# watsonyanghx/GAN_Lib_Tensorflow

Measured on AMD Instinct MI355X. Metric: images/sec (G+D step) SNGAN-ResNet CIFAR-10 bs=64, higher is better.
Workload: dtype bf16; 1 GPU; SNGAN ResNet CIFAR-10 32x32 bs=64 hinge: 1 G update (2x64 fakes) + 5 D updates (64 real + 64 fake) per step; global_batch=64, per_gpu_batch=64, parallelism=dp1, graphs=True, finite=True, collectives_in_graphs=False, grad_wire=fp32

## Files before the change

### gan_lib_tensorflow_amd/csrc/conv_igemm.hip

```cpp
#include "gank_common.h"
#ifdef GANK_TUNING
static __device__ int gank_stats_dbg = 0;
static void gank_stats_dbg_init() {
  static const int v = gank_tune("GANK_STATS_DBG", 0);
  static bool done = false;
  if (!done) { done = true; if (v) (void)hipMemcpyToSymbol(HIP_SYMBOL(gank_stats_dbg), &v, sizeof(int)); }
}
#else
static inline void gank_stats_dbg_init() {}
#endif
#include <stdlib.h>
#include <type_traits>

#ifndef GANK_KMODE
#define GANK_KMODE 0
#endif
#define IG_IN_ZEROINS2X 16
#define IG_IN_STRIDE2 32
#define IG_RES_UP2X 128

struct IgemmArgs {
  const bf16* x;
  const bf16* w;
  const float* bias;
  const bf16* res;
  const bf16* mask;
  bf16* y;
  int N, H, W;
  int Hin, Win;
  int Cin, Cout, CoutPad, Kpad;
  int ks, pad, taps;
  int M;
  int flags;
  float scale;
  int nsteps;
  int tiles_m, tiles_n;
  int shw, sw;
  int korder;
  int tiles_pp;
  float* stat_sums;
  int stat_n_per_group, stat_groups, stat_prezeroed;
  int phase_inner;
  const float* cbn_stats;
  const float* cbn_gamma;
  const float* cbn_beta;
  const int* cbn_labels;
  int cbn_n_per_group, cbn_n_labels;
  bf16* aux_out;
};

static int phase_inner_env() {
  static const int v = gank_tune("GANK_PHASE_INNER", 1);
  return v;
}

constexpr int LROW = 72;

template <int CTRL>
__device__ __forceinline__ float pp_dpp_add(float v) {
  return v + __builtin_bit_cast(float, __builtin_amdgcn_update_dpp(0, __builtin_bit_cast(int, v), CTRL, 0xF, 0xF, false));
}
__device__ __forceinline__ float pp_row_sum(float v) {
  v = pp_dpp_add<0xB1>(v);
  v = pp_dpp_add<0x4E>(v);
  v = pp_dpp_add<0x141>(v);
  v = pp_dpp_add<0x140>(v);
  return v;
}

template <bool WANT_D>
__device__ __forceinline__ void epi_tile_wide(const f32x16& acc, float scale, const float* __restrict__ bias, const bf16* __restrict__ mask_px,
                                              const bf16* __restrict__ res_px, bf16* __restrict__ y_px, int h, bool otanh, float (*d)[8]) {
#pragma unroll
  for (int q = 0; q < 2; q++) {
    const int c = 16 * q + 8 * h;
    float v[8];
    acc_widen(acc, q, scale, v);
    float bb[8] = {0.f, 0.f, 0.f, 0.f, 0.f, 0.f, 0.f, 0.f};
    if (bias) {
      const f32x4 b0 = *reinterpret_cast<const f32x4*>(bias + c), b1 = *reinterpret_cast<const f32x4*>(bias + c + 4);
#pragma unroll
      for (int e = 0; e < 4; e++) { bb[e] = b0[e]; bb[4 + e] = b1[e]; }
    }
#pragma unroll
    for (int e = 0; e < 8; e++) {
      if constexpr (WANT_D) d[q][e] = v[e];
      v[e] += bb[e];
    }
    if (mask_px) {
      const bf16x8 mk = *reinterpret_cast<const bf16x8*>(mask_px + c);
#pragma unroll
      for (int e = 0; e < 8; e++) {
        const bool on = bf2f(mk[e]) > 0.f;
        v[e] = on ? v[e] : 0.f;
        if constexpr (WANT_D) d[q][e] = on ? d[q][e] : -bb[e];
      }
    }
    if (res_px) {
      const bf16x8 rs = *reinterpret_cast<const bf16x8*>(res_px + c);
#pragma unroll
      for (int e = 0; e < 8; e++) {
        const float t = bf2f(rs[e]);
        v[e] += t;
        if constexpr (WANT_D) d[q][e] += t;
      }
    }
    bf16x8 out;
#pragma unroll
    for (int e = 0; e < 8; e++) out[e] = f2bf(otanh ? tanhf(v[e]) : v[e]);
    *reinterpret_cast<bf16x8*>(y_px + c) = out;
  }
}

template <int WM, int WN, int TM, int TN, bool PACKED, int PF, int MODE, bool STATS = false>
__global__ __launch_bounds__(WM* WN * 64) void conv_igemm_kernel(IgemmArgs a) {
  static_assert(!STATS || (!PACKED && TN * 16 <= 32), "statistics epilogue: plain operands, at most 32 channels per half-wave");
  constexpr int NT = WM * WN * 64;
  constexpr int BM = WM * TM * 32;
  constexpr int BN = WN * TN * 32;
  constexpr int CP = BM * 8 / NT;
  constexpr int CW = BN * 8 / NT;
  static_assert(CP >= 1 && CW >= 1, "tile too small for the thread count");
  static_assert(!PACKED || (PF == 1 && MODE == 0), "the packed path takes its flags at run time");

  extern __shared__ __attribute__((aligned(16))) char smem[];
  bf16* sP = reinterpret_cast<bf16*>(smem);
  bf16* sW = sP + 2 * BM * LROW;

  const int tid = threadIdx.x;
  const int lane = tid & 63, wave = tid >> 6;
  const int wave_m = wave % WM, wave_n = wave / WM;
  const int r = lane & 31, h = lane >> 5;

  const int nwg = a.tiles_m * a.tiles_n;
  const int lid = xcd_remap(blockIdx.x, nwg);
  const int tile_n = lid % a.tiles_n;
  int tile_m = lid / a.tiles_n;
  constexpr bool PHASE = !PACKED && (MODE & 4) != 0;
  int phase = 0;
  if constexpr (PHASE) {
    if (a.phase_inner) { phase = tile_m & 3; tile_m >>= 2; }
    else { phase = tile_m / a.tiles_pp; tile_m -= phase * a.tiles_pp; }
  }
  const int pad_h = PHASE ? 1 - (phase >> 1) : a.pad, pad_w = PHASE ? 1 - (phase & 1) : a.pad;

  const int st = (a.flags & IG_IN_STRIDE2) ? 2 : 1;
  const bool shr = PACKED ? (a.flags & (GANK_IN_UPSAMPLE2X | IG_IN_ZEROINS2X)) != 0 : (MODE & 2) != 0;
  const bool zins = (a.flags & IG_IN_ZEROINS2X) != 0;
  const bool inrelu = PACKED ? (a.flags & GANK_IN_RELU) != 0 : (MODE & 1) != 0;
  const int LH = shr ? 2 * a.Hin : a.Hin, LW = shr ? 2 * a.Win : a.Win;

  int p_base[CP], p_oh[CP], p_ow[CP];
#pragma unroll
  for (int j = 0; j < CP; j++) {
    const int q = tid + NT * j;
    const int m = tile_m * BM + (q >> 3);
    if (m < a.M) {
      int n, oh, ow;
      pix_decomp(m, a.H, a.W, a.shw, a.sw, n, oh, ow);
      p_base[j] = n * a.Hin * a.Win;
      p_oh[j] = oh * st;
      p_ow[j] = ow * st;
    } else {
      p_base[j] = 0;
      p_oh[j] = -(1 << 20);
      p_ow[j] = 0;
    }
  }

  u32x4 rP[PF][CP], rW[PF][CW];

  constexpr int OOB = 0x7FFFFFF0;
  const __amdgpu_buffer_rsrc_t rs_x = __builtin_amdgcn_make_buffer_rsrc(
      const_cast<bf16*>(a.x), 0, a.N * a.Hin * a.Win * a.Cin * 2, 0x00020000);
  const __amdgpu_buffer_rsrc_t rs_w = __builtin_amdgcn_make_buffer_rsrc(
      const_cast<bf16*>(a.w), 0, a.CoutPad * a.Kpad * 2 * (PHASE ? 4 : 1), 0x00020000);
  int p_off[CP];
  int w_off[CW];
#pragma unroll
  for (int j = 0; j < CP; j++)
    p_off[j] = ((p_base[j] + p_oh[j] * a.Win + p_ow[j]) * a.Cin + ((tid + NT * j) & 7) * 8) * 2;
#pragma unroll
  for (int j = 0; j < CW; j++) {
    const int q = tid + NT * j;
    w_off[j] = (((PHASE ? phase * a.CoutPad : 0) + tile_n * BN + (q >> 3)) * a.Kpad + (q & 7) * 8) * 2;
  }

  const int last = a.nsteps - 1;
  int cur = 0, cur_c0 = 0, cur_tap = 0, cur_dh = -pad_h, cur_dw = -pad_w;
  constexpr bool TAP_INNER = (GANK_KMODE & 1) != 0;
  constexpr int W_AUX = (GANK_KMODE >> 1) == 1 ? 2 : ((GANK_KMODE >> 1) == 2 ? 16 : 0);

  auto load_next = [&](u32x4 (&rP)[CP], u32x4 (&rW)[CW]) {
    if constexpr (!PACKED) {
      const int delta = ((cur_dh * a.Win + cur_dw) * a.Cin + cur_c0) * 2;
#pragma unroll
      for (int j = 0; j < CP; j++) {
        const int ih = p_oh[j] + cur_dh, iw = p_ow[j] + cur_dw;
        bool ok = (unsigned)ih < (unsigned)LH && (unsigned)iw < (unsigned)LW;
        int off;
        if constexpr ((MODE & 2) != 0) {
          if (zins) ok = ok && (((ih | iw) & 1) == 0);
          off = ((p_base[j] + (ih >> 1) * a.Win + (iw >> 1)) * a.Cin + cur_c0 + ((tid + NT * j) & 7) * 8) * 2;
        } else {
          off = p_off[j] + delta;
        }
        rP[j] = __builtin_amdgcn_raw_buffer_load_b128(rs_x, ok ? off : OOB, 0, 0);
      }
    } else {
      const int ktot = a.taps * a.Cin;
#pragma unroll
      for (int j = 0; j < CP; j++) {
        const int cc = (tid + NT * j) & 7;
        const int kb = cur * 64 + cc * 8;
        int tap = kb / a.Cin, ci = kb - tap * a.Cin;
        int th = tap / a.ks;
        int dh = th - a.pad, dw = tap - th * a.ks - a.pad;
        bf16x8 v;
#pragma unroll
        for (int e = 0; e < 8; e++) {
          float val = 0.f;
          if (kb + e < ktot) {
            int ih = p_oh[j] + dh, iw = p_ow[j] + dw;
            bool ok = (unsigned)ih < (unsigned)LH && (unsigned)iw < (unsigned)LW;
            if (zins) ok = ok && (((ih | iw) & 1) == 0);
            if (shr) { ih >>= 1; iw >>= 1; }
            if (ok) {
              val = bf2f(a.x[((long)(p_base[j] + ih * a.Win + iw)) * a.Cin + ci]);
              if (inrelu) val = fmaxf(val, 0.f);
            }
          }
          v[e] = f2bf(val);
          if (++ci == a.Cin) {
            ci = 0;
            if (++dw > a.ks - 1 - a.pad) { dw = -a.pad; dh++; }
          }
        }
        rP[j] = __builtin_bit_cast(u32x4, v);
      }
    }
    if constexpr (!PACKED) {
      const int wk = (cur_tap * a.Cin + cur_c0) * 2;
#pragma unroll
      for (int j = 0; j < CW; j++) rW[j] = __builtin_amdgcn_raw_buffer_load_b128(rs_w, w_off[j], wk, W_AUX);
      if (cur < last) {
        cur++;
        if constexpr (TAP_INNER) {
          cur_tap++;
          if (++cur_dw > a.ks - 1 - pad_w) { cur_dw = -pad_w; cur_dh++; }
          if (cur_tap >= a.taps) { cur_tap = 0; cur_dh = -pad_h; cur_dw = -pad_w; cur_c0 += 64; }
        } else {
          cur_c0 += 64;
          if (cur_c0 >= a.Cin) {
            cur_c0 = 0; cur_tap++;
            if (++cur_dw > a.ks - 1 - pad_w) { cur_dw = -pad_w; cur_dh++; }
          }
        }
      }
    } else {
#pragma unroll
      for (int j = 0; j < CW; j++) rW[j] = __builtin_amdgcn_raw_buffer_load_b128(rs_w, w_off[j], cur * 128, 0);
      if (cur < last) cur++;
    }
  };

  auto store_step = [&](int buf, u32x4 (&rP)[CP], u32x4 (&rW)[CW]) {
#pragma unroll
    for (int j = 0; j < CP; j++) {
      const int q = tid + NT * j;
      u32x4 v = rP[j];
      if constexpr (!PACKED && (MODE & 1) != 0) v = relu_bf16x8(v);
      *reinterpret_cast<u32x4*>(sP + (buf * BM + (q >> 3)) * LROW + (q & 7) * 8) = v;
    }
#pragma unroll
    for (int j = 0; j < CW; j++) {
      const int q = tid + NT * j;
      *reinterpret_cast<u32x4*>(sW + (buf * BN + (q >> 3)) * LROW + (q & 7) * 8) = rW[j];
    }
  };

  f32x16 acc[TN][TM];
#pragma unroll
  for (int i = 0; i < TN; i++)
#pragma unroll
    for (int j = 0; j < TM; j++)
#pragma unroll
      for (int e = 0; e < 16; e++) acc[i][j][e] = 0.f;

#pragma unroll
  for (int d = 0; d < PF; d++) load_next(rP[d], rW[d]);
  store_step(0, rP[0], rW[0]);
  __syncthreads();

  auto step = [&](int s, auto slot) {
    constexpr int D = decltype(slot)::value;
    const int buf = s & 1;
    if constexpr (PF > 1) {
      load_next(rP[D], rW[D]);
      if (s + 1 < a.nsteps) store_step(buf ^ 1, rP[(D + 1) % PF], rW[(D + 1) % PF]);
    }
    const bf16* pW = sW + (buf * BN + wave_n * TN * 32 + r) * LROW + h * 8;
    const bf16* pP = sP + (buf * BM + wave_m * TM * 32 + r) * LROW + h * 8;
#pragma unroll
    for (int kk = 0; kk < 4; kk++) {
      bf16x8 fa[TN], fb[TM];
#pragma unroll
      for (int i = 0; i < TN; i++) fa[i] = *reinterpret_cast<const bf16x8*>(pW + i * 32 * LROW + kk * 16);
#pragma unroll
      for (int j = 0; j < TM; j++) fb[j] = *reinterpret_cast<const bf16x8*>(pP + j * 32 * LROW + kk * 16);
#pragma unroll
      for (int i = 0; i < TN; i++)
#pragma unroll
        for (int j = 0; j < TM; j++)
          acc[i][j] = GANK_MFMA32(fa[i], fb[j], acc[i][j]);
    }
    if constexpr (PF == 1) {
      if (s + 1 < a.nsteps) {
        load_next(rP[0], rW[0]);
        store_step(buf ^ 1, rP[0], rW[0]);
      }
    }
    __syncthreads();
  };

  int s0 = 0;
  for (; s0 + PF <= a.nsteps; s0 += PF) {
    if constexpr (PF >= 1) step(s0 + 0, std::integral_constant<int, 0>{});
    if constexpr (PF >= 2) step(s0 + 1, std::integral_constant<int, 1 % PF>{});
    if constexpr (PF >= 3) step(s0 + 2, std::integral_constant<int, 2 % PF>{});
    if constexpr (PF >= 4) step(s0 + 3, std::integral_constant<int, 3 % PF>{});
  }
  if constexpr (PF >= 2) { if (s0 + 0 < a.nsteps) step(s0 + 0, std::integral_constant<int, 0>{}); }
  if constexpr (PF >= 3) { if (s0 + 1 < a.nsteps) step(s0 + 1, std::integral_constant<int, 1 % PF>{}); }
  if constexpr (PF >= 4) { if (s0 + 2 < a.nsteps) step(s0 + 2, std::integral_constant<int, 2 % PF>{}); }

  const bool vec = (a.Cout & 3) == 0;
  const bool wide = (a.Cout & 31) == 0;
  const bool otanh = (a.flags & GANK_OUT_TANH) != 0;
  float st1[STATS ? TN * 16 : 1], st2[STATS ? TN * 16 : 1];
  if constexpr (STATS) {
#pragma unroll
    for (int q = 0; q < TN * 16; q++) { st1[q] = 0.f; st2[q] = 0.f; }
  }
#pragma unroll
  for (int j = 0; j < TM; j++) {
    int m = tile_m * BM + (wave_m * TM + j) * 32 + r;
    if (m >= a.M) continue;
    if constexpr (PHASE) {
      int n_, y_, x_;
      pix_decomp(m, a.H, a.W, a.shw, a.sw, n_, y_, x_);
      m = (n_ * 2 * a.H + 2 * y_ + (phase >> 1)) * 2 * a.W + 2 * x_ + (phase & 1);
    }
    long mr = m;
    if (!PHASE && (a.flags & IG_RES_UP2X)) {
      int n_, y_, x_;
      pix_decomp(m, a.H, a.W, a.shw, a.sw, n_, y_, x_);
      mr = ((long)(n_ * (a.H >> 1) + (y_ >> 1))) * (a.W >> 1) + (x_ >> 1);
    }
    if (wide) {
#pragma unroll
      for (int i = 0; i < TN; i++) {
        const int ct = tile_n * BN + (wave_n * TN + i) * 32;
        float d[2][8];
        epi_tile_wide<STATS>(acc[i][j], a.scale, a.bias ? a.bias + ct : nullptr, a.mask ? a.mask + (long)m * a.Cout + ct : nullptr,
                             a.res ? a.res + mr * a.Cout + ct : nullptr, a.y + (long)m * a.Cout + ct, h, otanh, d);
        if constexpr (STATS) {
#pragma unroll
          for (int q = 0; q < 2; q++)
#pragma unroll
            for (int e = 0; e < 8; e++) { st1[i * 16 + q * 8 + e] += d[q][e]; st2[i * 16 + q * 8 + e] += d[q][e] * d[q][e]; }
        }
      }
      continue;
    }
#pragma unroll
    for (int i = 0; i < TN; i++) {
      const int co0 = tile_n * BN + (wave_n * TN + i) * 32 + 4 * h;
#pragma unroll
      for (int g = 0; g < 4; g++) {
        const int co = co0 + 8 * g;
        if (co >= a.Cout) continue;
        float v[4];
#pragma unroll
        for (int e = 0; e < 4; e++) v[e] = acc[i][j][4 * g + e] * a.scale;
        const long o = (long)m * a.Cout + co;
        if (vec) {
          f32x4 b = {0.f, 0.f, 0.f, 0.f};
          if (a.bias) {
            b = *reinterpret_cast<const f32x4*>(a.bias + co);
#pragma unroll
            for (int e = 0; e < 4; e++) v[e] += b[e];
          }
          if (a.mask) {
            const bf16x4 mk = *reinterpret_cast<const bf16x4*>(a.mask + o);
#pragma unroll
            for (int e = 0; e < 4; e++) v[e] = (bf2f(mk[e]) > 0.f) ? v[e] : 0.f;
          }
          if (a.res) {
            const bf16x4 rs = *reinterpret_cast<const bf16x4*>(a.res + mr * a.Cout + co);
#pragma unroll
            for (int e = 0; e < 4; e++) v[e] += bf2f(rs[e]);
          }
          bf16x4 out;
#pragma unroll
          for (int e = 0; e < 4; e++) out[e] = f2bf(otanh ? tanhf(v[e]) : v[e]);
          *reinterpret_cast<bf16x4*>(a.y + o) = out;
        } else {
#pragma unroll
          for (int e = 0; e < 4; e++) {
            if (co + e >= a.Cout) break;
            float t = v[e];
            if (a.bias) t += a.bias[co + e];
            if (a.mask) t = (bf2f(a.mask[o + e]) > 0.f) ? t : 0.f;
            if (a.res) t += bf2f(a.res[mr * a.Cout + co + e]);
            a.y[o + e] = f2bf(otanh ? tanhf(t) : t);
          }
        }
// ... 968 lines not shown
#pragma unroll
      for (int i = 0; i < 2; i++)
#pragma unroll
        for (int q = 0; q < 2; q++) *reinterpret_cast<bf16x8*>(line + i * 32 + 16 * q) = outl[i][q];
    }
    if constexpr (STATS) {
#pragma unroll
    for (int i = 0; i < 2; i++)
#pragma unroll
      for (int q = 0; q < 2; q++)
#pragma unroll
        for (int e = 0; e < 8; e++) {
          float s1 = pp_row_sum(st1[i][q][e]), s2 = pp_row_sum(st2[i][q][e]);
          s1 += __shfl_xor(s1, 16, 64);
          s2 += __shfl_xor(s2, 16, 64);
          const bool mine = r == (2 * i + q) * 8 + e;
          keep1 = mine ? s1 : keep1;
          keep2 = mine ? s2 : keep2;
        }
    }
  }
  if constexpr (STATS) {
    float* dst = a.stat_sums + ((long)(n / a.stat_n_per_group) * GANK_STAT_SLOTS + (blockIdx.x % GANK_STAT_SLOTS)) * 2 * a.Cout;
    const int ci = r >> 4, cq = (r >> 3) & 1, ce = r & 7;
    const int co = tile_n * 256 + (wn * 2 + ci) * 32 + 16 * cq + 8 * h + ce;
#ifdef GANK_TUNING
    if (gank_stats_dbg) return;
#endif
    atomicAdd(dst + co, keep1);
    atomicAdd(dst + a.Cout + co, keep2);
  }
#endif
}

static thread_local int tl_stats_done = 0;
__global__ void ig_zero_kernel(float* __restrict__ p, int n) {
  const int i = blockIdx.x * blockDim.x + threadIdx.x;
  if (i < n) p[i] = 0.f;
}

static void stats_zero(const IgemmArgs& a, hipStream_t s);
static int t128_min() {
  static const int v = gank_tune("GANK_IGEMM_T128_MIN", 192);
  return v;
}
static bool igemm_stats_ok(const IgemmArgs& a, int BM, int BN) {
  static const int env = gank_tune("GANK_IGEMM_STATS", 1);
  return env && a.stat_sums != nullptr && !(a.flags & GANK_OUT_TANH) && a.M % BM == 0 && a.Cout % BN == 0 &&
         ((long)a.stat_n_per_group * a.H * a.W) % BM == 0;
}
template <int MODE, int PW>
static int launch_pp(const IgemmArgs& a0, hipStream_t s) {
  IgemmArgs a = a0;
  const bool stats = a.stat_sums != nullptr;
  if (stats) { tl_stats_done = 1; stats_zero(a, s); }
  constexpr bool PHASE = (MODE & 4) != 0;
  const int tiles = a.N * (a.H / (256 / PW)) * (a.W / PW);
  a.tiles_pp = tiles;
  a.phase_inner = phase_inner_env();
  a.tiles_m = PHASE ? 4 * tiles : tiles;
  a.tiles_n = a.Cout / 256;
  if (PHASE) { a.Kpad = 4 * a.Cin; a.Hin = a.H; a.Win = a.W; }
  auto kern = stats ? conv_igemm_pp_kernel<MODE, PW, true> : conv_igemm_pp_kernel<MODE, PW, false>;
  if (stats) { GANK_MAX_DYNAMIC_LDS((conv_igemm_pp_kernel<MODE, PW, true>), PP_LDS_BYTES, "conv_igemm_pp"); }
  else { GANK_MAX_DYNAMIC_LDS((conv_igemm_pp_kernel<MODE, PW, false>), PP_LDS_BYTES, "conv_igemm_pp"); }
  static const std::string tag = gank_format("conv_igemm_pp_kernel<%d, %d>", MODE, PW);
  gank_prof_tag(0, tag.c_str());
  hipLaunchKernelGGL(kern, dim3(a.tiles_m * a.tiles_n), dim3(512), PP_LDS_BYTES, s, a);
  GANK_LAUNCH_OK("conv_igemm_pp");
  return 0;
}
static int pp_patch_width(int H, int W) { return (W % 32 == 0 && H % 8 == 0) ? 32 : (W % 16 == 0 && H % 16 == 0) ? 16 : 0; }
static int pp_env() {
  static const int v = gank_tune("GANK_IGEMM_PP", 2);
  return v;
}
static bool pp_enough_blocks(const IgemmArgs& a, int phases) {
  const int pw = pp_patch_width(a.H, a.W);
  return pw != 0 && (long)phases * a.N * (a.H / (256 / pw)) * (a.W / pw) * (a.Cout / 256) >= 224;
}
static bool pp_phase_ok(const IgemmArgs& a) {
  return pp_env() >= 2 && a.Cout % 256 == 0 && a.Cin % 32 == 0 && pp_enough_blocks(a, 4);
}
static int launch_pp_phase(const IgemmArgs& a, hipStream_t s) {
  const bool relu = (a.flags & GANK_IN_RELU) != 0;
  if (pp_patch_width(a.H, a.W) == 32) return relu ? launch_pp<5, 32>(a, s) : launch_pp<4, 32>(a, s);
  return relu ? launch_pp<5, 16>(a, s) : launch_pp<4, 16>(a, s);
}

template <int MODE, int BN>
static int launch_patch(const IgemmArgs& a0, hipStream_t s) {
  IgemmArgs a = a0;
  a.tiles_m = a.N * (a.H / 8) * (a.W / 16);
  a.tiles_n = a.CoutPad / BN;
  const size_t lds = ((size_t)10 * HROWP + (size_t)2 * BN * LROW) * sizeof(bf16);
  auto kern = conv_igemm_patch_kernel<MODE, BN>;
  GANK_MAX_DYNAMIC_LDS(kern, (int)lds, "conv_igemm_patch");
  static const std::string tag = gank_format("conv_igemm_patch_kernel<%d, %d>", MODE, BN);
  gank_prof_tag(0, tag.c_str());
  hipLaunchKernelGGL(kern, dim3(a.tiles_m * a.tiles_n), dim3(256), lds, s, a);
  GANK_LAUNCH_OK("conv_igemm_patch");
  return 0;
}

template <int WM, int WN, int TM, int TN, bool PACKED, int PF, int MODE>
static int launch_cfg(const IgemmArgs& a0, hipStream_t s) {
  IgemmArgs a = a0;
  constexpr int BM = WM * TM * 32, BN = WN * TN * 32;
  a.tiles_m = cdiv(a.M, BM);
  a.tiles_n = a.CoutPad / BN;
  const size_t lds = (size_t)2 * (BM + BN) * LROW * sizeof(bf16);
  static const std::string tag = gank_format("conv_igemm_kernel<%d, %d, %d, %d, %s, %d, %d>", WM, WN, TM, TN, PACKED ? "true" : "false", PF, MODE);
  gank_prof_tag(0, tag.c_str());
  if constexpr (!PACKED && MODE == 0 && TN * 16 <= 32) {
    if (igemm_stats_ok(a, BM, BN)) {
      auto kern = conv_igemm_kernel<WM, WN, TM, TN, PACKED, PF, MODE, true>;
      GANK_MAX_DYNAMIC_LDS(kern, (int)lds, "conv_igemm");
      tl_stats_done = 1;
      stats_zero(a, s);
      hipLaunchKernelGGL(kern, dim3(a.tiles_m * a.tiles_n), dim3(WM * WN * 64), lds, s, a);
      GANK_LAUNCH_OK("conv_igemm");
      return 0;
    }
  }
  auto kern = conv_igemm_kernel<WM, WN, TM, TN, PACKED, PF, MODE>;
  GANK_MAX_DYNAMIC_LDS(kern, (int)lds, "conv_igemm");
  hipLaunchKernelGGL(kern, dim3(a.tiles_m * a.tiles_n), dim3(WM * WN * 64), lds, s, a);
  GANK_LAUNCH_OK("conv_igemm");
  return 0;
}

template <int WM, int WN, int TM, int TN, int PF>
static int launch_phase(const IgemmArgs& a0, hipStream_t s) {
  IgemmArgs a = a0;
  constexpr int BM = WM * TM * 32, BN = WN * TN * 32;
  a.tiles_pp = cdiv(a.M, BM);
  a.phase_inner = phase_inner_env();
  a.tiles_m = 4 * a.tiles_pp;
  a.tiles_n = a.CoutPad / BN;
  const size_t lds = (size_t)2 * (BM + BN) * LROW * sizeof(bf16);
  static const std::string tag = gank_format("conv_igemm_kernel<%d, %d, %d, %d, false, %d, 4>", WM, WN, TM, TN, PF);
  gank_prof_tag(0, tag.c_str());
  if constexpr (TN * 16 <= 32) {
    if (igemm_stats_ok(a, BM, BN)) {
      auto kern = conv_igemm_kernel<WM, WN, TM, TN, false, PF, 4, true>;
      GANK_MAX_DYNAMIC_LDS(kern, (int)lds, "conv_igemm");
      tl_stats_done = 1;
      stats_zero(a, s);
      hipLaunchKernelGGL(kern, dim3(a.tiles_m * a.tiles_n), dim3(WM * WN * 64), lds, s, a);
      GANK_LAUNCH_OK("conv_igemm_phase");
      return 0;
    }
  }
  auto kern = conv_igemm_kernel<WM, WN, TM, TN, false, PF, 4>;
  GANK_MAX_DYNAMIC_LDS(kern, (int)lds, "conv_igemm");
  hipLaunchKernelGGL(kern, dim3(a.tiles_m * a.tiles_n), dim3(WM * WN * 64), lds, s, a);
  GANK_LAUNCH_OK("conv_igemm_phase");
  return 0;
}

template <int WM, int WN, int TM, int TN, int PF>
static int launch_mode(const IgemmArgs& a, hipStream_t s) {
  const int mode = ((a.flags & GANK_IN_RELU) ? 1 : 0) | ((a.flags & (GANK_IN_UPSAMPLE2X | IG_IN_ZEROINS2X)) ? 2 : 0);
  switch (mode) {
    case 0: return launch_cfg<WM, WN, TM, TN, false, PF, 0>(a, s);
    case 1: return launch_cfg<WM, WN, TM, TN, false, PF, 1>(a, s);
    case 2: return launch_cfg<WM, WN, TM, TN, false, PF, 2>(a, s);
    default: return launch_cfg<WM, WN, TM, TN, false, PF, 3>(a, s);
  }
}

int gank_igemm_dispatch(IgemmArgs a, hipStream_t s) {
  GANK_REQUIRE(a.x && a.w && a.y, "conv_igemm: null pointer");
  GANK_REQUIRE(a.N > 0 && a.H > 0 && a.W > 0 && a.Cin > 0 && a.Cout > 0, "conv_igemm: bad shape");
  GANK_REQUIRE(a.ks >= 1 && a.ks <= 7, "conv_igemm: unsupported filter size %d", a.ks);
  GANK_REQUIRE((long)a.N * a.Hin * a.Win * a.Cin < (1L << 30) && (long)a.N * a.H * a.W * a.Cout < (1L << 40), "conv_igemm: tensor too large (32-bit byte offsets)");
  a.taps = a.ks * a.ks;
  a.CoutPad = roundup(a.Cout, 32);
  a.Kpad = roundup(a.taps * a.Cin, 64);
  a.nsteps = a.Kpad / 64;
  a.M = a.N * a.H * a.W;
  a.sw = log2_or_neg(a.W);
  a.shw = log2_or_neg(a.H * a.W);
  const bool packed = (a.Cin % 64) != 0;
  const double flops = 2.0 * a.M * (double)a.Cout * a.taps * a.Cin;
  gank_prof_begin(0, flops, s, 2.0 * ((double)a.N * a.Hin * a.Win * a.Cin + (double)a.taps * a.Cin * a.Cout + (double)a.M * a.Cout +
                                      (a.res ? (double)a.M * a.Cout / ((a.flags & IG_RES_UP2X) ? 4.0 : 1.0) : 0.0) + (a.mask ? (double)a.M * a.Cout : 0.0)));
  int rc;
  const long tiles128 = (long)cdiv(a.M, 128) * (a.CoutPad / 128);
  static const int ko_env = gank_tune("GANK_IGEMM_KORDER", 0);
  a.korder = ko_env;
  static const int pf_env = gank_tune("GANK_IGEMM_PF", 0);
  static const int patch_env = gank_tune("GANK_IGEMM_PATCH", 1);
  const bool patch_geom = patch_env && !packed && a.ks == 3 && a.pad == 1 &&
                          !(a.flags & (GANK_IN_UPSAMPLE2X | IG_IN_ZEROINS2X | IG_IN_STRIDE2)) &&
                          a.W % 16 == 0 && a.H % 8 == 0 && a.Hin == a.H && a.Win == a.W;
  const bool patch_ok = patch_geom && (a.Cout % 4) == 0 && a.CoutPad % 128 == 0;
  const bool patch32_ok = patch_geom && a.CoutPad == 32;
  const bool narrow_ok = !(a.flags & IG_RES_UP2X) && a.Cin == 3 && (a.ks == 1 || a.ks == 3) && a.pad == (a.ks - 1) / 2 && a.CoutPad % 128 == 0 && a.Cout % 4 == 0 &&
                         !(a.flags & (GANK_IN_UPSAMPLE2X | IG_IN_ZEROINS2X | IG_IN_STRIDE2)) && a.Hin == a.H && a.Win == a.W;
  const bool pp_ok = pp_env() && patch_geom && a.Cout % 256 == 0 && a.Kpad == a.taps * a.Cin && pp_enough_blocks(a, 1) &&
                     (pp_env() >= 2 || pp_patch_width(a.H, a.W) == 32);
  if (narrow_ok) {
    rc = a.ks == 3 ? launch_narrow_in<3, 3>(a, s) : launch_narrow_in<1, 3>(a, s);
  } else if (pp_ok) {
    const bool relu = (a.flags & GANK_IN_RELU) != 0;
    if (pp_patch_width(a.H, a.W) == 32) rc = relu ? launch_pp<1, 32>(a, s) : launch_pp<0, 32>(a, s);
    else rc = relu ? launch_pp<1, 16>(a, s) : launch_pp<0, 16>(a, s);
  } else if (patch_ok) {
    rc = (a.flags & GANK_IN_RELU) ? launch_patch<1, 128>(a, s) : launch_patch<0, 128>(a, s);
  } else if (patch32_ok && few_ok(a)) {
    rc = (a.flags & GANK_IN_RELU) ? launch_few<1>(a, s) : launch_few<0>(a, s);
  } else if (patch32_ok) {
    rc = (a.flags & GANK_IN_RELU) ? launch_patch<1, 32>(a, s) : launch_patch<0, 32>(a, s);
  } else if (packed) {
    if (a.CoutPad % 64 == 0) rc = launch_cfg<2, 2, 1, 1, true, 1, 0>(a, s);
    else rc = launch_cfg<4, 1, 2, 1, true, 1, 0>(a, s);
#ifdef GANK_TUNING
  } else if (a.CoutPad % 128 == 0 && tiles128 >= t128_min() && pf_env >= 20) {
    if (pf_env == 20) rc = launch_mode<4, 2, 2, 2, 1>(a, s);
    else if (pf_env == 22 && a.CoutPad % 256 == 0) rc = launch_mode<2, 4, 2, 2, 2>(a, s);
    else if (pf_env == 23 && a.CoutPad % 256 == 0) rc = launch_mode<4, 2, 2, 4, 2>(a, s);
    else rc = launch_mode<4, 2, 2, 2, 2>(a, s);
  } else if (a.CoutPad % 128 == 0 && tiles128 >= t128_min() && (pf_env == 1 || pf_env == 3)) {
    rc = pf_env == 1 ? launch_mode<2, 2, 2, 2, 1>(a, s) : launch_mode<2, 2, 2, 2, 3>(a, s);
  } else if (a.CoutPad % 64 == 0 && !(a.CoutPad % 128 == 0 && tiles128 >= t128_min()) && (pf_env == 1 || pf_env == 11 || pf_env == 12 || pf_env == 3)) {
    rc = (pf_env == 1 || pf_env == 11) ? launch_mode<2, 2, 1, 1, 1>(a, s) : launch_mode<2, 2, 1, 1, 2>(a, s);
#endif
  } else if (a.CoutPad % 128 == 0 && tiles128 >= t128_min()) {
    rc = launch_mode<2, 2, 2, 2, 2>(a, s);
  } else if (a.CoutPad % 64 == 0) {
    rc = launch_mode<2, 2, 1, 1, 4>(a, s);
  } else {
    rc = launch_mode<4, 1, 2, 1, 2>(a, s);
  }
  gank_prof_end(0, s);
  return rc;
}

static int stats_setup(IgemmArgs& a, float* stat_sums, int groups, int N, int Cout, hipStream_t s, int flags) {
  tl_stats_done = 0;
  if (!stat_sums) return 0;
  gank_stats_dbg_init();
  a.stat_prezeroed = (flags & GANK_STATS_PREZEROED) != 0;
  GANK_REQUIRE(groups > 0 && N % groups == 0, "conv statistics: batch %d not divisible by %d towers", N, groups);
  a.stat_sums = stat_sums;
  a.stat_n_per_group = N / groups;
  a.stat_groups = groups;
  return 0;
}
static void stats_zero(const IgemmArgs& a, hipStream_t s) {
  if (a.stat_prezeroed) return;
  const int n = a.stat_groups * GANK_STAT_SLOTS * 2 * a.Cout;
  hipLaunchKernelGGL(ig_zero_kernel, dim3((n + 255) / 256), dim3(256), 0, s, a.stat_sums, n);
}

static int conv2d_fprop_impl(const void* x, const void* wf, const float* bias, const void* residual,
                             const void* relu_ref, void* y, int N, int H, int W, int Cin, int Cout, int ksize,
                             int flags, float scale, float* stat_sums, int groups, void* stream) {
  GANK_REQUIRE(ksize % 2 == 1, "conv2d_fprop: even filter sizes are not on this path (ksize=%d)", ksize);
  GANK_REQUIRE(!(flags & GANK_IN_UPSAMPLE2X) || (H % 2 == 0 && W % 2 == 0), "conv2d_fprop: upsample needs even output size");
  IgemmArgs a{};
  a.x = (const bf16*)x; a.w = (const bf16*)wf; a.bias = bias; a.res = (const bf16*)residual;
  a.mask = (const bf16*)relu_ref; a.y = (bf16*)y;
  a.N = N; a.H = H; a.W = W;
  const bool up = flags & GANK_IN_UPSAMPLE2X;
  a.Hin = up ? H / 2 : H; a.Win = up ? W / 2 : W;
  a.Cin = Cin; a.Cout = Cout; a.ks = ksize; a.pad = (ksize - 1) / 2;
  a.flags = (flags & (GANK_IN_UPSAMPLE2X | GANK_IN_RELU | GANK_OUT_TANH)) |
            ((flags & GANK_RES_UPSAMPLE2X) ? IG_RES_UP2X : 0);
  GANK_REQUIRE(!(flags & GANK_RES_UPSAMPLE2X) || (residual && H % 2 == 0 && W % 2 == 0), "conv2d_fprop: RES_UPSAMPLE2X needs a residual and even output size");
  a.scale = scale;
  if (stats_setup(a, stat_sums, groups, N, Cout, (hipStream_t)stream, flags)) return 1;
  return gank_igemm_dispatch(a, (hipStream_t)stream);
}

extern "C" int gank_conv2d_fprop(const void* x, const void* wf, const float* bias, const void* residual,
                                 const void* relu_ref, void* y, int N, int H, int W, int Cin, int Cout, int ksize,
                                 int flags, float scale, void* stream) {
  return conv2d_fprop_impl(x, wf, bias, residual, relu_ref, y, N, H, W, Cin, Cout, ksize, flags, scale, nullptr, 0, stream);
}
extern "C" int gank_conv2d_fprop_stats(const void* x, const void* wf, const float* bias, const void* residual,
                                       const void* relu_ref, void* y, int N, int H, int W, int Cin, int Cout, int ksize,
                                       int flags, float scale, float* stat_sums, int groups, int* produced, void* stream) {
  GANK_REQUIRE(stat_sums && produced, "conv2d_fprop_stats: null statistics pointers");
  const int rc = conv2d_fprop_impl(x, wf, bias, residual, relu_ref, y, N, H, W, Cin, Cout, ksize, flags, scale, stat_sums, groups, stream);
  *produced = tl_stats_done;
  return rc;
}

extern "C" int gank_cbn_relu_conv3x3_fprop(const void* x, const int32_t* labels, const float* gamma, const float* beta, const float* stats,
                                           const void* wf, const float* bias, void* y, int N, int H, int W, int Cin, int Cout,
                                           int groups, int n_labels, int flags, void* stream) {
  GANK_REQUIRE(x && labels && gamma && beta && stats && wf && y, "cbn_relu_conv3x3_fprop: null pointer");
  GANK_REQUIRE(groups > 0 && N % groups == 0 && n_labels > 0, "cbn_relu_conv3x3_fprop: batch %d / %d towers", N, groups);
  GANK_REQUIRE(Cin % 64 == 0 && W % 16 == 0 && H % 8 == 0, "cbn_relu_conv3x3_fprop: needs Cin %% 64 == 0, W %% 16 == 0, H %% 8 == 0");
  IgemmArgs a{};
// ... 41 lines not shown
  IgemmArgs a{}, b{};
  a.x = (const bf16*)x; a.w = (const bf16*)wf1; a.bias = bias1; a.y = (bf16*)y1;
  a.N = N; a.H = H; a.W = W; a.Hin = H; a.Win = W; a.Cin = 3; a.Cout = Cout1; a.ks = 3; a.pad = 1; a.scale = 1.f;
  a.taps = 9; a.CoutPad = Cout1; a.Kpad = roundup(27, 64); a.nsteps = 1;
  a.M = N * H * W; a.sw = log2_or_neg(W); a.shw = log2_or_neg(H * W);
  a.tiles_m = cdiv(a.M, 128); a.tiles_n = a.CoutPad / 128;
  { static const int ko_env = gank_tune("GANK_IGEMM_KORDER", 0); a.korder = ko_env; }
  const int Hp = H / 2, Wp = W / 2;
  b.x = (const bf16*)x; b.w = (const bf16*)wfs; b.bias = biass; b.y = (bf16*)ys; b.aux_out = (bf16*)pooled;
  b.N = N; b.H = Hp; b.W = Wp; b.Hin = H; b.Win = W; b.Cin = 3; b.Cout = Couts; b.ks = 1; b.pad = 0; b.scale = 1.f;
  b.taps = 1; b.CoutPad = Couts; b.Kpad = roundup(3, 64); b.nsteps = 1;
  b.M = N * Hp * Wp; b.sw = log2_or_neg(Wp); b.shw = log2_or_neg(Hp * Wp);
  b.tiles_m = cdiv(b.M, 128); b.tiles_n = b.CoutPad / 128;
  b.korder = 0;
  hipStream_t s = (hipStream_t)stream;
  const int blocks_a = a.tiles_m * a.tiles_n, blocks_b = b.tiles_m * b.tiles_n;
  gank_prof_begin(0, 2.0 * a.M * (double)Cout1 * 27 + 2.0 * b.M * (double)Couts * 3, s,
                  2.0 * ((double)a.M * 3 + 27.0 * Cout1 + (double)a.M * Cout1 + 3.0 * Couts + (double)b.M * Couts));
  gank_prof_tag(0, "conv_narrow_in_pair_kernel");
  hipLaunchKernelGGL(conv_narrow_in_pair_kernel, dim3(blocks_a + blocks_b), dim3(256), 0, s, a, b, blocks_a);
  gank_prof_end(0, s);
  GANK_LAUNCH_OK("image_conv_pair_fprop");
  return 0;
}

extern "C" int gank_conv2d_dgrad(const void* dy, const void* wd, const void* residual, const void* relu_ref, void* dx,
                                 int N, int H, int W, int Cin, int Cout, int ksize, int flags, float scale, void* stream) {
  GANK_REQUIRE(ksize % 2 == 1, "conv2d_dgrad: even filter sizes are not on this path (ksize=%d)", ksize);
  IgemmArgs a{};
  a.x = (const bf16*)dy; a.w = (const bf16*)wd; a.bias = nullptr; a.res = (const bf16*)residual;
  a.mask = (const bf16*)relu_ref; a.y = (bf16*)dx;
  a.N = N; a.H = H; a.W = W;
  const bool up = flags & GANK_IN_UPSAMPLE2X;
  a.Hin = up ? H / 2 : H; a.Win = up ? W / 2 : W;
  a.Cin = Cout; a.Cout = Cin; a.ks = ksize; a.pad = (ksize - 1) / 2;
  a.flags = (flags & (GANK_IN_UPSAMPLE2X | GANK_IN_RELU));
  a.scale = scale;
  return gank_igemm_dispatch(a, (hipStream_t)stream);
}


extern "C" int gank_conv2d_general_fprop(const void* x, const void* wf, const float* bias, void* y, int N, int Hin, int Win,
                                         int Hout, int Wout, int Cin, int Cout, int ksize, int stride, int pad, int flags, void* stream) {
  GANK_REQUIRE(stride == 1 || stride == 2, "conv2d_general_fprop: stride %d (1 or 2)", stride);
  GANK_REQUIRE(pad >= 0 && pad < ksize, "conv2d_general_fprop: pad %d outside [0, ksize)", pad);
  GANK_REQUIRE(!((flags & GANK_IN_UPSAMPLE2X) && stride == 2), "conv2d_general_fprop: upsampled input with stride 2");
  GANK_REQUIRE(Hin > 0 && Win > 0 && Hout > 0 && Wout > 0, "conv2d_general_fprop: bad sizes");
  IgemmArgs a{};
  a.x = (const bf16*)x; a.w = (const bf16*)wf; a.bias = bias; a.y = (bf16*)y;
  a.N = N; a.H = Hout; a.W = Wout; a.Hin = Hin; a.Win = Win;
  a.Cin = Cin; a.Cout = Cout; a.ks = ksize; a.pad = pad;
  a.flags = (flags & (GANK_IN_UPSAMPLE2X | GANK_IN_RELU | GANK_OUT_TANH)) | (stride == 2 ? IG_IN_STRIDE2 : 0);
  a.scale = 1.f;
  return gank_igemm_dispatch(a, (hipStream_t)stream);
}
extern "C" int gank_conv2d_general_dgrad(const void* dy, const void* wd, const void* relu_ref, void* dx, int N, int Hx, int Wx,
                                         int Hdy, int Wdy, int Cin, int Cout, int ksize, int pad, void* stream) {
  GANK_REQUIRE(pad >= 0 && pad < ksize, "conv2d_general_dgrad: pad %d outside [0, ksize)", pad);
  IgemmArgs a{};
  a.x = (const bf16*)dy; a.w = (const bf16*)wd; a.mask = (const bf16*)relu_ref; a.y = (bf16*)dx;
  a.N = N; a.H = Hx; a.W = Wx; a.Hin = Hdy; a.Win = Wdy;
  a.Cin = Cout; a.Cout = Cin; a.ks = ksize; a.pad = ksize - 1 - pad;
  a.scale = 1.f;
  return gank_igemm_dispatch(a, (hipStream_t)stream);
}

static int upconv3x3_fprop_impl(const void* x, const void* wph, const float* bias, const void* residual, void* y,
                                int N, int Hl, int Wl, int Cin, int Cout, int flags, float* stat_sums, int groups, void* stream) {
  GANK_REQUIRE(Cin % 64 == 0, "upconv3x3_fprop: Cin must be a multiple of 64 (got %d)", Cin);
  IgemmArgs a{};
  a.x = (const bf16*)x; a.w = (const bf16*)wph; a.bias = bias; a.res = (const bf16*)residual; a.y = (bf16*)y;
  a.N = N; a.H = Hl; a.W = Wl; a.Hin = Hl; a.Win = Wl;
  a.Cin = Cin; a.Cout = Cout; a.ks = 2; a.pad = 0;
  a.flags = flags & GANK_OUT_TANH;
  a.scale = 1.f;
  hipStream_t s = (hipStream_t)stream;
  a.taps = 4; a.CoutPad = roundup(Cout, 32); a.Kpad = 4 * Cin; a.nsteps = a.Kpad / 64;
  a.M = N * Hl * Wl; a.sw = log2_or_neg(Wl); a.shw = log2_or_neg(Hl * Wl);
  GANK_REQUIRE((long)N * Hl * Wl * Cin < (1L << 30) && (long)a.M * 4 * Cout < (1L << 31), "upconv3x3_fprop: tensor too large");
  if (stats_setup(a, stat_sums, groups, N, Cout, s, flags)) return 1;
  gank_prof_begin(0, 2.0 * a.M * 4.0 * (double)Cout * 4 * Cin, s, 2.0 * ((double)a.M * Cin + 16.0 * Cin * Cout + 4.0 * a.M * Cout + (residual ? 4.0 * a.M * Cout : 0.0)));
  int rc;
  const long tiles128 = 4L * cdiv(a.M, 128) * (a.CoutPad / 128);
  if (pp_phase_ok(a)) rc = launch_pp_phase(a, s);
  else if (patch_phase_ok(a)) rc = launch_patch_phase<4>(a, s);
  else if (a.CoutPad % 128 == 0 && tiles128 >= t128_min()) rc = launch_phase<2, 2, 2, 2, 2>(a, s);
  else if (a.CoutPad % 64 == 0) rc = launch_phase<2, 2, 1, 1, 4>(a, s);
  else rc = launch_phase<4, 1, 2, 1, 2>(a, s);
  gank_prof_end(0, s);
  return rc;
}

extern "C" int gank_upconv3x3_fprop(const void* x, const void* wph, const float* bias, const void* residual, void* y,
                                    int N, int Hl, int Wl, int Cin, int Cout, int flags, void* stream) {
  return upconv3x3_fprop_impl(x, wph, bias, residual, y, N, Hl, Wl, Cin, Cout, flags, nullptr, 0, stream);
}
extern "C" int gank_upconv3x3_fprop_stats(const void* x, const void* wph, const float* bias, const void* residual, void* y,
                                          int N, int Hl, int Wl, int Cin, int Cout, int flags, float* stat_sums, int groups, int* produced,
                                          void* stream) {
  GANK_REQUIRE(stat_sums && produced, "upconv3x3_fprop_stats: null statistics pointers");
  const int rc = upconv3x3_fprop_impl(x, wph, bias, residual, y, N, Hl, Wl, Cin, Cout, flags, stat_sums, groups, stream);
  *produced = tl_stats_done;
  return rc;
}

extern "C" int gank_upconv3x3_dgrad(const void* dy, const void* wd4, const void* relu_ref, void* dx, int N, int Hl, int Wl,
                                    int Cin, int Cout, void* stream) {
  IgemmArgs a{};
  a.x = (const bf16*)dy; a.w = (const bf16*)wd4; a.mask = (const bf16*)relu_ref; a.y = (bf16*)dx;
  a.N = N; a.H = Hl; a.W = Wl; a.Hin = 2 * Hl; a.Win = 2 * Wl;
  a.Cin = Cout; a.Cout = Cin; a.ks = 4; a.pad = 1;
  a.flags = IG_IN_STRIDE2;
  a.scale = 1.f;
  return gank_igemm_dispatch(a, (hipStream_t)stream);
}

extern "C" int gank_convpool3x3_fprop(const void* x, const void* wp4, const float* bias, const void* residual, void* y,
                                      int N, int Hp, int Wp, int Cin, int Cout, int flags, void* stream) {
  IgemmArgs a{};
  a.x = (const bf16*)x; a.w = (const bf16*)wp4; a.bias = bias; a.res = (const bf16*)residual; a.y = (bf16*)y;
  a.N = N; a.H = Hp; a.W = Wp; a.Hin = 2 * Hp; a.Win = 2 * Wp;
  a.Cin = Cin; a.Cout = Cout; a.ks = 4; a.pad = 1;
  a.flags = IG_IN_STRIDE2 | (flags & GANK_IN_RELU);
  a.scale = 1.f;
  return gank_igemm_dispatch(a, (hipStream_t)stream);
}

extern "C" int gank_convpool3x3_dgrad(const void* dy, const void* wphd, const void* relu_ref, void* dx, int N, int Hp, int Wp,
                                      int Cin, int Cout, void* stream) {
  GANK_REQUIRE(Cout % 64 == 0, "convpool3x3_dgrad: Cout must be a multiple of 64 (got %d)", Cout);
  IgemmArgs a{};
  a.x = (const bf16*)dy; a.w = (const bf16*)wphd; a.mask = (const bf16*)relu_ref; a.y = (bf16*)dx;
  a.N = N; a.H = Hp; a.W = Wp; a.Hin = Hp; a.Win = Wp;
  a.Cin = Cout; a.Cout = Cin; a.ks = 2; a.pad = 0;
  a.flags = 0;
  a.scale = 1.f;
  hipStream_t s = (hipStream_t)stream;
  a.taps = 4; a.CoutPad = roundup(Cin, 32); a.Kpad = 4 * Cout; a.nsteps = a.Kpad / 64;
  a.M = N * Hp * Wp; a.sw = log2_or_neg(Wp); a.shw = log2_or_neg(Hp * Wp);
  GANK_REQUIRE((long)N * Hp * Wp * Cout < (1L << 30) && (long)a.M * 4 * Cin < (1L << 31), "convpool3x3_dgrad: tensor too large");
  gank_prof_begin(0, 2.0 * a.M * 4.0 * (double)Cin * 4 * Cout, s, 2.0 * ((double)a.M * Cout + 16.0 * Cin * Cout + 4.0 * a.M * Cin + (relu_ref ? 4.0 * a.M * Cin : 0.0)));
  int rc;
  const long tiles128 = 4L * cdiv(a.M, 128) * (a.CoutPad / 128);
  if (pp_phase_ok(a)) rc = launch_pp_phase(a, s);
  else if (patch_phase_ok(a)) rc = launch_patch_phase<4>(a, s);
  else if (a.CoutPad % 128 == 0 && tiles128 >= t128_min()) rc = launch_phase<2, 2, 2, 2, 2>(a, s);
  else if (a.CoutPad % 64 == 0) rc = launch_phase<2, 2, 1, 1, 4>(a, s);
  else rc = launch_phase<4, 1, 2, 1, 2>(a, s);
  gank_prof_end(0, s);
  return rc;
}

static int deconv_pad_before(int ks) { int t = ks - 2; if (t < 0) t = 0; return t / 2; }

extern "C" int gank_deconv2d_fprop(const void* x, const void* wz, const float* bias, void* y, int N, int H, int W,
                                   int Cin, int Cout, int ksize, void* stream) {
  IgemmArgs a{};
  a.x = (const bf16*)x; a.w = (const bf16*)wz; a.bias = bias; a.y = (bf16*)y;
  a.N = N; a.H = 2 * H; a.W = 2 * W; a.Hin = H; a.Win = W;
  a.Cin = Cin; a.Cout = Cout; a.ks = ksize;
  a.pad = ksize - 1 - deconv_pad_before(ksize);
  a.flags = IG_IN_ZEROINS2X;
  a.scale = 1.f;
  return gank_igemm_dispatch(a, (hipStream_t)stream);
}

extern "C" int gank_deconv2d_dgrad(const void* dy, const void* wfz, void* dx, int N, int H, int W, int Cin, int Cout,
                                   int ksize, void* stream) {
  IgemmArgs a{};
  a.x = (const bf16*)dy; a.w = (const bf16*)wfz; a.y = (bf16*)dx;
  a.N = N; a.H = H; a.W = W; a.Hin = 2 * H; a.Win = 2 * W;
  a.Cin = Cout; a.Cout = Cin; a.ks = ksize; a.pad = deconv_pad_before(ksize);
  a.flags = IG_IN_STRIDE2;
  a.scale = 1.f;
  return gank_igemm_dispatch(a, (hipStream_t)stream);
}
```

Before: 58860 images/sec.

## Add 128-channel K-step with wave-split reduction for small upconv GEMMs

Adds a KC=128 template option to the implicit-GEMM conv kernel, plus a wave-split mode in which each of four waves handles a 32-channel slice of the K-step over the whole 64x64 tile. The partial accumulators are then summed through LDS at the end. It is routed in for 4x4/8x8 upconv forward and dgrad layers with Cin a multiple of 128, where the output tile grid is small. The aim is to halve the number of K steps and barriers, and to keep all waves busy despite few output tiles. In exchange it uses more LDS, adds a reduction pass, and adds more kernel instantiations.

After: 58800 images/sec, median of 2. No clear change (-0.1%).

```diff
diff --git a/gan_lib_tensorflow_amd/csrc/conv_igemm.hip b/gan_lib_tensorflow_amd/csrc/conv_igemm.hip
--- a/gan_lib_tensorflow_amd/csrc/conv_igemm.hip
+++ b/gan_lib_tensorflow_amd/csrc/conv_igemm.hip
@@ -18,6 +18,7 @@
 #define IG_IN_ZEROINS2X 16
 #define IG_IN_STRIDE2 32
 #define IG_RES_UP2X 128
+#define IG_SMALL_UPCONV 1024
 
 struct IgemmArgs {
   const bf16* x;
@@ -112,20 +113,26 @@
   }
 }
 
-template <int WM, int WN, int TM, int TN, bool PACKED, int PF, int MODE, bool STATS = false>
+template <int WM, int WN, int TM, int TN, bool PACKED, int PF, int MODE, bool STATS = false, int KC = 64, bool KSPLIT = false>
 __global__ __launch_bounds__(WM* WN * 64) void conv_igemm_kernel(IgemmArgs a) {
   static_assert(!STATS || (!PACKED && TN * 16 <= 32), "statistics epilogue: plain operands, at most 32 channels per half-wave");
+  static_assert(KC == 64 || (KC == 128 && !PACKED), "K-step: 64 channels, or 128 on the plain operands");
+  static_assert(!KSPLIT || (KC == 128 && WM == 2 && WN == 2 && TM == 1 && TN == 1), "wave-split K-step: 2 x 2 waves, 32 channels each");
   constexpr int NT = WM * WN * 64;
   constexpr int BM = WM * TM * 32;
   constexpr int BN = WN * TN * 32;
-  constexpr int CP = BM * 8 / NT;
-  constexpr int CW = BN * 8 / NT;
+  constexpr int KCH = KC / 8;
+  constexpr int LR = KC + 8;
+  constexpr int CP = BM * KCH / NT;
+  constexpr int CW = BN * KCH / NT;
+  constexpr int GM = KSPLIT ? WM * TM : TM, GN = KSPLIT ? WN * TN : TN;
   static_assert(CP >= 1 && CW >= 1, "tile too small for the thread count");
   static_assert(!PACKED || (PF == 1 && MODE == 0), "the packed path takes its flags at run time");
+  static_assert(!KSPLIT || 4 * GM * GN * 64 * 64 <= 2 * (BM + BN) * LR * 2, "the partial tiles are summed in the staging buffers");
 
   extern __shared__ __attribute__((aligned(16))) char smem[];
   bf16* sP = reinterpret_cast<bf16*>(smem);
-  bf16* sW = sP + 2 * BM * LROW;
+  bf16* sW = sP + 2 * BM * LR;
 
   const int tid = threadIdx.x;
   const int lane = tid & 63, wave = tid >> 6;
@@ -154,7 +161,7 @@
 #pragma unroll
   for (int j = 0; j < CP; j++) {
     const int q = tid + NT * j;
-    const int m = tile_m * BM + (q >> 3);
+    const int m = tile_m * BM + (q / KCH);
     if (m < a.M) {
       int n, oh, ow;
       pix_decomp(m, a.H, a.W, a.shw, a.sw, n, oh, ow);
@@ -179,11 +186,11 @@
   int w_off[CW];
 #pragma unroll
   for (int j = 0; j < CP; j++)
-    p_off[j] = ((p_base[j] + p_oh[j] * a.Win + p_ow[j]) * a.Cin + ((tid + NT * j) & 7) * 8) * 2;
+    p_off[j] = ((p_base[j] + p_oh[j] * a.Win + p_ow[j]) * a.Cin + ((tid + NT * j) % KCH) * 8) * 2;
 #pragma unroll
   for (int j = 0; j < CW; j++) {
     const int q = tid + NT * j;
-    w_off[j] = (((PHASE ? phase * a.CoutPad : 0) + tile_n * BN + (q >> 3)) * a.Kpad + (q & 7) * 8) * 2;
+    w_off[j] = (((PHASE ? phase * a.CoutPad : 0) + tile_n * BN + (q / KCH)) * a.Kpad + (q % KCH) * 8) * 2;
   }
 
   const int last = a.nsteps - 1;
@@ -201,7 +208,7 @@
         int off;
         if constexpr ((MODE & 2) != 0) {
           if (zins) ok = ok && (((ih | iw) & 1) == 0);
-          off = ((p_base[j] + (ih >> 1) * a.Win + (iw >> 1)) * a.Cin + cur_c0 + ((tid + NT * j) & 7) * 8) * 2;
+          off = ((p_base[j] + (ih >> 1) * a.Win + (iw >> 1)) * a.Cin + cur_c0 + ((tid + NT * j) % KCH) * 8) * 2;
         } else {
           off = p_off[j] + delta;
         }
@@ -248,9 +255,9 @@
         if constexpr (TAP_INNER) {
           cur_tap++;
           if (++cur_dw > a.ks - 1 - pad_w) { cur_dw = -pad_w; cur_dh++; }
-          if (cur_tap >= a.taps) { cur_tap = 0; cur_dh = -pad_h; cur_dw = -pad_w; cur_c0 += 64; }
+          if (cur_tap >= a.taps) { cur_tap = 0; cur_dh = -pad_h; cur_dw = -pad_w; cur_c0 += KC; }
         } else {
-          cur_c0 += 64;
+          cur_c0 += KC;
           if (cur_c0 >= a.Cin) {
             cur_c0 = 0; cur_tap++;
             if (++cur_dw > a.ks - 1 - pad_w) { cur_dw = -pad_w; cur_dh++; }
@@ -270,20 +277,20 @@
       const int q = tid + NT * j;
       u32x4 v = rP[j];
       if constexpr (!PACKED && (MODE & 1) != 0) v = relu_bf16x8(v);
-      *reinterpret_cast<u32x4*>(sP + (buf * BM + (q >> 3)) * LROW + (q & 7) * 8) = v;
+      *reinterpret_cast<u32x4*>(sP + (buf * BM + (q / KCH)) * LR + (q % KCH) * 8) = v;
     }
 #pragma unroll
     for (int j = 0; j < CW; j++) {
       const int q = tid + NT * j;
-      *reinterpret_cast<u32x4*>(sW + (buf * BN + (q >> 3)) * LROW + (q & 7) * 8) = rW[j];
+      *reinterpret_cast<u32x4*>(sW + (buf * BN + (q / KCH)) * LR + (q % KCH) * 8) = rW[j];
     }
   };
 
-  f32x16 acc[TN][TM];
-#pragma unroll
-  for (int i = 0; i < TN; i++)
-#pragma unroll
-    for (int j = 0; j < TM; j++)
+  f32x16 acc[GN][GM];
+#pragma unroll
+  for (int i = 0; i < GN; i++)
+#pragma unroll
+    for (int j = 0; j < GM; j++)
 #pragma unroll
       for (int e = 0; e < 16; e++) acc[i][j][e] = 0.f;
 
@@ -299,19 +306,19 @@
       load_next(rP[D], rW[D]);
       if (s + 1 < a.nsteps) store_step(buf ^ 1, rP[(D + 1) % PF], rW[(D + 1) % PF]);
     }
-    const bf16* pW = sW + (buf * BN + wave_n * TN * 32 + r) * LROW + h * 8;
-    const bf16* pP = sP + (buf * BM + wave_m * TM * 32 + r) * LROW + h * 8;
-#pragma unroll
-    for (int kk = 0; kk < 4; kk++) {
-      bf16x8 fa[TN], fb[TM];
-#pragma unroll
-      for (int i = 0; i < TN; i++) fa[i] = *reinterpret_cast<const bf16x8*>(pW + i * 32 * LROW + kk * 16);
-#pragma unroll
-      for (int j = 0; j < TM; j++) fb[j] = *reinterpret_cast<const bf16x8*>(pP + j * 32 * LROW + kk * 16);
-#pragma unroll
-      for (int i = 0; i < TN; i++)
-#pragma unroll
-        for (int j = 0; j < TM; j++)
+    const bf16* pW = sW + (buf * BN + (KSPLIT ? 0 : wave_n * TN * 32) + r) * LR + h * 8 + (KSPLIT ? wave * 32 : 0);
+    const bf16* pP = sP + (buf * BM + (KSPLIT ? 0 : wave_m * TM * 32) + r) * LR + h * 8 + (KSPLIT ? wave * 32 : 0);
+#pragma unroll
+    for (int kk = 0; kk < (KSPLIT ? 2 : KC / 16); kk++) {
+      bf16x8 fa[GN], fb[GM];
+#pragma unroll
+      for (int i = 0; i < GN; i++) fa[i] = *reinterpret_cast<const bf16x8*>(pW + i * 32 * LR + kk * 16);
+#pragma unroll
+      for (int j = 0; j < GM; j++) fb[j] = *reinterpret_cast<const bf16x8*>(pP + j * 32 * LR + kk * 16);
+#pragma unroll
+      for (int i = 0; i < GN; i++)
+#pragma unroll
+        for (int j = 0; j < GM; j++)
           acc[i][j] = GANK_MFMA32(fa[i], fb[j], acc[i][j]);
     }
     if constexpr (PF == 1) {
@@ -333,6 +340,31 @@
   if constexpr (PF >= 2) { if (s0 + 0 < a.nsteps) step(s0 + 0, std::integral_constant<int, 0>{}); }
   if constexpr (PF >= 3) { if (s0 + 1 < a.nsteps) step(s0 + 1, std::integral_constant<int, 1 % PF>{}); }
   if constexpr (PF >= 4) { if (s0 + 2 < a.nsteps) step(s0 + 2, std::integral_constant<int, 2 % PF>{}); }
+
+  if constexpr (KSPLIT) {
+    f32x4* red = reinterpret_cast<f32x4*>(smem);
+#pragma unroll
+    for (int i = 0; i < GN; i++)
+#pragma unroll
+      for (int j = 0; j < GM; j++)
+#pragma unroll
+        for (int g = 0; g < 4; g++)
+          red[((wave * GN * GM + i * GM + j) * 4 + g) * 64 + lane] = f32x4{acc[i][j][4 * g], acc[i][j][4 * g + 1], acc[i][j][4 * g + 2], acc[i][j][4 * g + 3]};
+    __syncthreads();
+    const int t = wave_n * GM + wave_m;
+#pragma unroll
+    for (int g = 0; g < 4; g++) {
+      f32x4 v = red[((0 * GN * GM + t) * 4 + g) * 64 + lane];
+#pragma unroll
+      for (int w = 1; w < 4; w++) {
+        const f32x4 u = red[((w * GN * GM + t) * 4 + g) * 64 + lane];
+#pragma unroll
+        for (int e = 0; e < 4; e++) v[e] += u[e];
+      }
+#pragma unroll
+      for (int e = 0; e < 4; e++) acc[0][0][4 * g + e] = v[e];
+    }
+  }
 
   const bool vec = (a.Cout & 3) == 0;
   const bool wide = (a.Cout & 31) == 0;
@@ -1467,6 +1499,11 @@
 static bool pp_phase_ok(const IgemmArgs& a) {
   return pp_env() >= 2 && a.Cout % 256 == 0 && a.Cin % 32 == 0 && pp_enough_blocks(a, 4);
 }
+static int small_upconv_mode(const IgemmArgs& a) {
+  static const int env = gank_tune("GANK_IGEMM_UPCONV_K128", 1);
+  const bool geom = a.H == a.W && (a.H == 4 || a.H == 8) && a.Cin % 128 == 0 && a.CoutPad % 64 == 0 && a.Kpad == a.taps * a.Cin;
+  return geom ? env : 0;
+}
 static int launch_pp_phase(const IgemmArgs& a, hipStream_t s) {
   const bool relu = (a.flags & GANK_IN_RELU) != 0;
   if (pp_patch_width(a.H, a.W) == 32) return relu ? launch_pp<5, 32>(a, s) : launch_pp<4, 32>(a, s);
@@ -1488,18 +1525,20 @@
   return 0;
 }
 
-template <int WM, int WN, int TM, int TN, bool PACKED, int PF, int MODE>
+template <int WM, int WN, int TM, int TN, bool PACKED, int PF, int MODE, int KC = 64, bool KSPLIT = false>
 static int launch_cfg(const IgemmArgs& a0, hipStream_t s) {
   IgemmArgs a = a0;
   constexpr int BM = WM * TM * 32, BN = WN * TN * 32;
   a.tiles_m = cdiv(a.M, BM);
   a.tiles_n = a.CoutPad / BN;
-  const size_t lds = (size_t)2 * (BM + BN) * LROW * sizeof(bf16);
-  static const std::string tag = gank_format("conv_igemm_kernel<%d, %d, %d, %d, %s, %d, %d>", WM, WN, TM, TN, PACKED ? "true" : "false", PF, MODE);
+  a.nsteps = a.Kpad / KC;
+  const size_t lds = (size_t)2 * (BM + BN) * (KC + 8) * sizeof(bf16);
+  static const std::string tag = gank_format("conv_igemm_kernel<%d, %d, %d, %d, %s, %d, %d%s>", WM, WN, TM, TN, PACKED ? "true" : "false", PF, MODE,
+                                             KC == 64 ? "" : KSPLIT ? ", k128 wave-split" : ", k128");
   gank_prof_tag(0, tag.c_str());
   if constexpr (!PACKED && MODE == 0 && TN * 16 <= 32) {
     if (igemm_stats_ok(a, BM, BN)) {
-      auto kern = conv_igemm_kernel<WM, WN, TM, TN, PACKED, PF, MODE, true>;
+      auto kern = conv_igemm_kernel<WM, WN, TM, TN, PACKED, PF, MODE, true, KC, KSPLIT>;
       GANK_MAX_DYNAMIC_LDS(kern, (int)lds, "conv_igemm");
       tl_stats_done = 1;
       stats_zero(a, s);
@@ -1508,14 +1547,14 @@
       return 0;
     }
   }
-  auto kern = conv_igemm_kernel<WM, WN, TM, TN, PACKED, PF, MODE>;
+  auto kern = conv_igemm_kernel<WM, WN, TM, TN, PACKED, PF, MODE, false, KC, KSPLIT>;
   GANK_MAX_DYNAMIC_LDS(kern, (int)lds, "conv_igemm");
   hipLaunchKernelGGL(kern, dim3(a.tiles_m * a.tiles_n), dim3(WM * WN * 64), lds, s, a);
   GANK_LAUNCH_OK("conv_igemm");
   return 0;
 }
 
-template <int WM, int WN, int TM, int TN, int PF>
+template <int WM, int WN, int TM, int TN, int PF, int KC = 64, bool KSPLIT = false>
 static int launch_phase(const IgemmArgs& a0, hipStream_t s) {
   IgemmArgs a = a0;
   constexpr int BM = WM * TM * 32, BN = WN * TN * 32;
@@ -1523,12 +1562,14 @@
   a.phase_inner = phase_inner_env();
   a.tiles_m = 4 * a.tiles_pp;
   a.tiles_n = a.CoutPad / BN;
-  const size_t lds = (size_t)2 * (BM + BN) * LROW * sizeof(bf16);
-  static const std::string tag = gank_format("conv_igemm_kernel<%d, %d, %d, %d, false, %d, 4>", WM, WN, TM, TN, PF);
+  a.nsteps = a.Kpad / KC;
+  const size_t lds = (size_t)2 * (BM + BN) * (KC + 8) * sizeof(bf16);
+  static const std::string tag = gank_format("conv_igemm_kernel<%d, %d, %d, %d, false, %d, 4%s>", WM, WN, TM, TN, PF,
+                                             KC == 64 ? "" : KSPLIT ? ", k128 wave-split" : ", k128");
   gank_prof_tag(0, tag.c_str());
   if constexpr (TN * 16 <= 32) {
     if (igemm_stats_ok(a, BM, BN)) {
-      auto kern = conv_igemm_kernel<WM, WN, TM, TN, false, PF, 4, true>;
+      auto kern = conv_igemm_kernel<WM, WN, TM, TN, false, PF, 4, true, KC, KSPLIT>;
       GANK_MAX_DYNAMIC_LDS(kern, (int)lds, "conv_igemm");
       tl_stats_done = 1;
       stats_zero(a, s);
@@ -1537,7 +1578,7 @@
       return 0;
     }
   }
-  auto kern = conv_igemm_kernel<WM, WN, TM, TN, false, PF, 4>;
+  auto kern = conv_igemm_kernel<WM, WN, TM, TN, false, PF, 4, false, KC, KSPLIT>;
   GANK_MAX_DYNAMIC_LDS(kern, (int)lds, "conv_igemm");
   hipLaunchKernelGGL(kern, dim3(a.tiles_m * a.tiles_n), dim3(WM * WN * 64), lds, s, a);
   GANK_LAUNCH_OK("conv_igemm_phase");
@@ -1598,6 +1639,9 @@
     rc = (a.flags & GANK_IN_RELU) ? launch_few<1>(a, s) : launch_few<0>(a, s);
   } else if (patch32_ok) {
     rc = (a.flags & GANK_IN_RELU) ? launch_patch<1, 32>(a, s) : launch_patch<0, 32>(a, s);
+  } else if ((a.flags & IG_SMALL_UPCONV) && !(a.flags & GANK_IN_RELU) && (small_upconv_mode(a) & 1) &&
+             ((small_upconv_mode(a) & 2) || !(a.CoutPad % 128 == 0 && tiles128 >= t128_min()))) {
+    rc = (small_upconv_mode(a) & 4) ? launch_cfg<2, 2, 1, 1, false, 2, 0, 128, false>(a, s) : launch_cfg<2, 2, 1, 1, false, 2, 0, 128, true>(a, s);
   } else if (packed) {
     if (a.CoutPad % 64 == 0) rc = launch_cfg<2, 2, 1, 1, true, 1, 0>(a, s);
     else rc = launch_cfg<4, 1, 2, 1, true, 1, 0>(a, s);
@@ -1805,8 +1849,11 @@
   gank_prof_begin(0, 2.0 * a.M * 4.0 * (double)Cout * 4 * Cin, s, 2.0 * ((double)a.M * Cin + 16.0 * Cin * Cout + 4.0 * a.M * Cout + (residual ? 4.0 * a.M * Cout : 0.0)));
   int rc;
   const long tiles128 = 4L * cdiv(a.M, 128) * (a.CoutPad / 128);
+  const int k128 = small_upconv_mode(a);
   if (pp_phase_ok(a)) rc = launch_pp_phase(a, s);
   else if (patch_phase_ok(a)) rc = launch_patch_phase<4>(a, s);
+  else if ((k128 & 1) && ((k128 & 2) || !(a.CoutPad % 128 == 0 && tiles128 >= t128_min())))
+    rc = (k128 & 4) ? launch_phase<2, 2, 1, 1, 2, 128, false>(a, s) : launch_phase<2, 2, 1, 1, 2, 128, true>(a, s);
   else if (a.CoutPad % 128 == 0 && tiles128 >= t128_min()) rc = launch_phase<2, 2, 2, 2, 2>(a, s);
   else if (a.CoutPad % 64 == 0) rc = launch_phase<2, 2, 1, 1, 4>(a, s);
   else rc = launch_phase<4, 1, 2, 1, 2>(a, s);
@@ -1833,7 +1880,7 @@
   a.x = (const bf16*)dy; a.w = (const bf16*)wd4; a.mask = (const bf16*)relu_ref; a.y = (bf16*)dx;
   a.N = N; a.H = Hl; a.W = Wl; a.Hin = 2 * Hl; a.Win = 2 * Wl;
   a.Cin = Cout; a.Cout = Cin; a.ks = 4; a.pad = 1;
-  a.flags = IG_IN_STRIDE2;
+  a.flags = IG_IN_STRIDE2 | IG_SMALL_UPCONV;
   a.scale = 1.f;
   return gank_igemm_dispatch(a, (hipStream_t)stream);
 }
```
